# jorge-menjivar/tekken-rs

Measured on AMD Instinct MI355X. Metric: input MB/s tokenized (whole node), higher is better.
Workload: dtype u8

## Files before the change

tekken-rs_amd/csrc/tk_flat_args.h:

```cpp
#ifndef TK_FLAT_ARGS_H
#define TK_FLAT_ARGS_H
#include <stdint.h>

#include "tk_counters.h"
#include "tk_tables.h"

#define TKF_W 32
#define TKF_REGION (64 * TKF_W)
#define TKF_HL 32
#define TKF_HR 64
#define TKF_COMMIT (TKF_REGION - TKF_HL - TKF_HR)
#define TKF_LONGCAP 256u
#define TKF_STRIDE (TKF_COMMIT + 64 + TKF_LONGCAP)
#define TKF_OWN (TKF_COMMIT + TKF_HR)
#define TKF_MISSOFF0 0u
#define TKF_MISSOFF1 (TKF_OWN / 2u)
#define TKF_MISSOFF2 (TKF_MISSOFF1 + (TKF_OWN + 8u) / 9u)
#define TKF_MISSOFF3 (TKF_MISSOFF2 + (TKF_OWN + 16u) / 17u)
#define TKF_MISSCAP ((TKF_MISSOFF3 + (TKF_OWN + 32u) / 33u + 7u) & ~7u)
#define TKF_POSBITS 11
#define TKF_REC(pos, len, slot) ((pos) | ((len) << TKF_POSBITS) | ((slot) << (TKF_POSBITS + 7)))
#define TKF_REC_POS(rec) ((rec) & ((1u << TKF_POSBITS) - 1u))
#define TKF_REC_LEN(rec) (((rec) >> TKF_POSBITS) & 127u)
#define TKF_REC_SLOT(rec) ((rec) >> (TKF_POSBITS + 7))
#define TKF_HOLE 0xFFFFFFFFu

struct TkFlatLongRec {
    uint64_t pos;
    uint32_t chunk;
    uint32_t slot;
    uint32_t len;
    uint32_t reserved;
};

#define TKF_LREC_FRAG 0x80000000u

struct TkFlatArgs {
    const uint8_t* bytes;
    const uint64_t* doc_offs;
    uint64_t n_docs, n_bytes, n_chunks;
    const uint32_t* first_doc;
    uint32_t* tmp;
    uint32_t* kcount;
    uint32_t* lstart;
    uint32_t* miss_list;
    uint32_t* miss_count;
    const uint64_t* miss_prefix;
    uint32_t* wave_first;
    uint32_t* wave_first_wide;
    uint32_t* holes;
    uint32_t* flags;
    TkFlatLongRec* long_recs;
    uint32_t* long_count;
    uint32_t long_cap;
    int long_merge128;
    const uint32_t* long_ctl;
    uint32_t* cut_list;
    const uint32_t* cut_count;
    uint32_t* late_list;
    uint32_t* late_count;
    tk_memo_entry* memo_tab;
    uint32_t memo_mask;
    int memo_probe;
    uint32_t memo_epoch;
    uint32_t* memo_hits;
    tk_memo_entry* memo_log;
    uint32_t* memo_log_counts;
    uint32_t memo_log_per_wave, memo_log_waves;
    uint8_t* dbg_starts;
    int pattern;
    int dbg_ablate;
    TkTablesView t;
};

#endif
```

tekken-rs_amd/csrc/tk_flat_impl.h:

```cpp
#ifndef TK_FLAT_IMPL_H
#define TK_FLAT_IMPL_H
#include <stdint.h>

#include "tk_encode_impl.h"
#include "tk_flat_args.h"

#define TKF_WM 0xFFFFFFFFu
#define TKF_LOGW 5
#define TKF_TOPBIT 0x80000000u
#define TKF_NHL (TKF_HL / TKF_W)
#ifndef TKF_LISTCAP
#define TKF_LISTCAP 1056
#endif
#define TKF_MAXPIECES (TKF_LISTCAP - 2)

#define TKF_L_LIST 0
#define TKF_L_DS (TKF_L_LIST + TKF_LISTCAP / 2)
#define TKF_L_PS (TKF_L_DS + 64)
#define TKF_L_PFX (TKF_L_PS + 64)
#define TKF_L_BAD (TKF_L_PFX + 64)
#define TKF_L_BPFX (TKF_L_BAD + 64)
#define TKF_WALKOFF 192
#define TKF_WALKCAP (2 * (TKF_LISTCAP / 2 - TKF_WALKOFF))
#define TKF_L_CL TKF_L_LIST
#define TKF_L_KM (TKF_L_BPFX + 64)
#define TKF_L_MEMO TKF_L_KM
#define TKF_L_TXT (TKF_L_KM + 17 * 4)
#define TKF_L_CONST (TKF_L_TXT + TKF_REGION / 4 + 4)
#define TKF_LDS_WORDS (TKF_L_CONST + 8)
#define TKF_L_FS TKF_LDS_WORDS
#define TKF_LDS_WORDS_CUT (TKF_LDS_WORDS + 64)


TK_DEV uint32_t tkf_shl(uint32_t x, int k) { return (uint32_t)((((uint64_t)x << 32) | (uint64_t)wv_dn1(x)) >> (32 - k)); }
TK_DEV uint32_t tkf_shr(uint32_t x, int k) { return (uint32_t)((((uint64_t)wv_up1(x) << 32) | (uint64_t)x) >> k); }
TK_DEV uint32_t tkf_shl_any(uint32_t x, int k, int lane) {
    const int q = k >> TKF_LOGW, r = k & (TKF_W - 1);
    const int s1 = lane - q, s2 = lane - q - 1;
    uint32_t v1 = wv_shfl(x, s1 & 63), v2 = wv_shfl(x, s2 & 63);
    if (s1 < 0) v1 = 0;
    if (s2 < 0) v2 = 0;
    return (uint32_t)((((uint64_t)v1 << TKF_W) | (uint64_t)v2) >> (TKF_W - r)) & TKF_WM;
}
TK_DEV uint32_t tkf_shr_any(uint32_t x, int k, int lane) {
    const int q = k >> TKF_LOGW, r = k & (TKF_W - 1);
    const int s1 = lane + q, s2 = lane + q + 1;
    uint32_t v1 = wv_shfl(x, s1 & 63), v2 = wv_shfl(x, s2 & 63);
    if (s1 > 63) v1 = 0;
    if (s2 > 63) v2 = 0;
    return (uint32_t)((((uint64_t)v2 << TKF_W) | (uint64_t)v1) >> r) & TKF_WM;
}
TK_DEV bool tkf_any(uint32_t x) { return wv_ballot(x != 0u) != 0ull; }

TK_DEV uint32_t tkf_add(uint32_t a, uint32_t b) {
    const uint32_t t = a + b;
    const uint64_t G = wv_ballot(t < a);
    const uint64_t P = wv_ballot((t & TKF_WM) == TKF_WM);
    const uint64_t x = G | P;
    const uint64_t cin = (x + G) ^ x ^ G;
    return (t + (wv_inverse_ballot(cin) ? 1u : 0u)) & TKF_WM;
}
TK_DEV uint32_t tkf_ripple(uint32_t run, uint32_t seeds) { return (tkf_add(run, seeds) ^ run) & run; }
TK_DEV uint32_t tkf_land(uint32_t run, uint32_t seeds) { return tkf_add(run, seeds) & ~run & TKF_WM; }

TK_DEV uint32_t tkf_scan_excl(uint32_t v, int lane, uint32_t* total) {
    (void)lane;
    const uint32_t x = wv_scan_incl_u32(v);
    *total = wv_readlane(x, 63);
    return x - v;
}

struct TkfClass {
    uint32_t L, N, S, NL, SP, AP, HI, STMD, RV, E, LL;
    uint32_t U8C, LEAD, C5, BF;
    uint32_t UP, SL, X, M;
    uint32_t F2, F3;
    bool nmb;
};

TK_DEV void tkf_transpose8(uint32_t& lo, uint32_t& hi) {
    uint32_t t;
    t = ((lo >> 7) ^ lo) & 0x00AA00AAu; lo ^= t ^ (t << 7);
    t = ((hi >> 7) ^ hi) & 0x00AA00AAu; hi ^= t ^ (t << 7);
    t = ((lo >> 14) ^ lo) & 0x0000CCCCu; lo ^= t ^ (t << 14);
    t = ((hi >> 14) ^ hi) & 0x0000CCCCu; hi ^= t ^ (t << 14);
    t = (((lo >> 28) | (hi << 4)) ^ lo) & 0xF0F0F0F0u;
    lo ^= t ^ (t << 28);
    hi ^= t >> 4;
}

TK_DEV TkfClass tkf_classify(const uint32_t* x) {
    uint32_t a_lo = x[0], a_hi = x[1], b_lo = x[2], b_hi = x[3];
    tkf_transpose8(a_lo, a_hi);
    tkf_transpose8(b_lo, b_hi);
    uint32_t c_lo = x[4], c_hi = x[5], d_lo = x[6], d_hi = x[7];
    tkf_transpose8(c_lo, c_hi);
    tkf_transpose8(d_lo, d_hi);
    const uint32_t u0 = wv_perm(b_lo, a_lo, 0x05010400u), u1 = wv_perm(b_lo, a_lo, 0x07030602u);
    const uint32_t v0 = wv_perm(d_lo, c_lo, 0x05010400u), v1 = wv_perm(d_lo, c_lo, 0x07030602u);
    const uint32_t p0 = wv_perm(v0, u0, 0x05040100u), p1 = wv_perm(v0, u0, 0x07060302u);
    const uint32_t p2 = wv_perm(v1, u1, 0x05040100u), p3 = wv_perm(v1, u1, 0x07060302u);
    const uint32_t u2 = wv_perm(b_hi, a_hi, 0x05010400u), u3 = wv_perm(b_hi, a_hi, 0x07030602u);
    const uint32_t v2 = wv_perm(d_hi, c_hi, 0x05010400u), v3 = wv_perm(d_hi, c_hi, 0x07030602u);
    const uint32_t p4 = wv_perm(v2, u2, 0x05040100u), p5 = wv_perm(v2, u2, 0x07060302u);
// ... 372 lines not shown
                        } else if (b0b < 0xF0u) {
                            if ((b1 & 0xC0u) == 0x80u && (b2 & 0xC0u) == 0x80u) {
                                cp = ((b0b & 0x0Fu) << 12) | ((b1 & 0x3Fu) << 6) | (b2 & 0x3Fu); clen = 3;
                            }
                        } else if (b0b < 0xF8u) {
                            if ((b1 & 0xC0u) == 0x80u && (b2 & 0xC0u) == 0x80u && (b3 & 0xC0u) == 0x80u) {
                                cp = ((b0b & 0x07u) << 18) | ((b1 & 0x3Fu) << 12) | ((b2 & 0x3Fu) << 6) | (b3 & 0x3Fu); clen = 4;
                            }
                        }
                        const uint32_t q = cp < 0x10000u ? cp : 0u;
                        uint32_t cw = t.uc_bmp[q >> 4];
                        uint32_t cls = (cw >> (2u * (q & 15u))) & 3u;
                        if (cp >= 0x10000u) cls = cp == 0xFFFFFFFFu ? (uint32_t)TK_CLS_O : tk_uc_class(t, cp);
                        if (cls != TK_CLS_O) {
                            const uint32_t wi = p >> TKF_LOGW, sh = p & (TKF_W - 1);
                            const uint64_t bits = (uint64_t)((1u << clen) - 1u) << sh;
                            wv_lds_or(cl + (cls - 1u) * 64u + wi, (uint32_t)(bits & TKF_WM));
                            if ((bits >> TKF_W) && wi < 63u) wv_lds_or(cl + (cls - 1u) * 64u + wi + 1u, (uint32_t)(bits >> TKF_W));
                            if (cls == TK_CLS_N) nmb = true;
                        }
                    }
                }
            }
        }
        while (!dealt && wv_ballot(w != 0u)) {
            if (w) {
                if (PAT) {
                    const int i = __builtin_ctz(w);
                    w &= w - 1u;
                    uint32_t clen;
                    const uint32_t cp = decode(i, &clen);
                    uint32_t cls = TK_CLS_O, extra = 0;
                    if (cp != 0xFFFFFFFFu) {
                        const uint32_t c2 = tk_uc_class2(t, cp);
                        cls = c2 == 1u || c2 == 2u ? TK_CLS_L : c2 == 5u ? TK_CLS_N : c2 == 6u ? TK_CLS_S : TK_CLS_O;
                        extra = c2 == 1u ? 1u : c2 == 3u ? 2u : c2 == 4u ? 3u : 0u;
                    }
                    mark(i, clen, cls, extra);
                } else {
                    const int i0 = __builtin_ctz(w);
                    w &= w - 1u;
                    const bool two = w != 0u;
                    const int i1 = two ? __builtin_ctz(w) : i0;
                    w &= w - 1u;
                    uint32_t l0, l1;
                    const uint32_t cp0 = decode(i0, &l0), cp1 = decode(i1, &l1);
                    const uint32_t q0 = cp0 < 0x10000u ? cp0 : 0u, q1 = cp1 < 0x10000u ? cp1 : 0u;
                    uint32_t w0 = t.uc_bmp[q0 >> 4], w1 = t.uc_bmp[q1 >> 4];
                    WV_PIN(w0); WV_PIN(w1);
                    uint32_t c0 = (w0 >> (2u * (q0 & 15u))) & 3u, c1 = (w1 >> (2u * (q1 & 15u))) & 3u;
                    if (cp0 >= 0x10000u) c0 = cp0 == 0xFFFFFFFFu ? (uint32_t)TK_CLS_O : tk_uc_class(t, cp0);
                    if (cp1 >= 0x10000u) c1 = cp1 == 0xFFFFFFFFu ? (uint32_t)TK_CLS_O : tk_uc_class(t, cp1);
                    mark(i0, l0, c0, 0u);
                    if (two) mark(i1, l1, c1, 0u);
                }
            }
        }
        wv_lds_sync();
        m.L |= cl[lane];
        m.N |= cl[64 + lane];
        m.S |= cl[128 + lane];
        m.nmb = wv_ballot(nmb) != 0ull;
        if (PAT) {
            m.UP |= cl[192 + lane];
            m.X = cl[256 + lane];
            m.M = cl[320 + lane];
        }
    }
    if (TKF_ABL(a, 16)) {
        const uint32_t v = m.L + m.N + m.S + m.NL + m.SP + m.AP + m.HI + m.STMD + m.RV + m.E + m.LL;
        if (lane == 0) {
            a.kcount[c] = v == 0xFFFFFFFFu ? 1u : 0u;
            for (int k = 0; k < 4; ++k) a.miss_count[k * a.n_chunks + c] = 0u;
        }
        return false;
    }

    lds[TKF_L_DS + lane] = 0u;
    lds[TKF_L_BAD + lane] = 0u;
    wv_lds_sync();
    const uint64_t fd = WV_KARGS(TkFlatArgs, a).first_doc[c];
    bool starts_at_r1 = false;
    {
        const auto& ka = WV_KARGS(TkFlatArgs, a);
        for (uint64_t base = fd;; base += 64) {
            const uint64_t d = base + (uint64_t)lane;
            int64_t s = INT64_MAX;
            if (d <= ka.n_docs) s = (int64_t)ka.doc_offs[d];
            const bool in = s < r1;
            if (in) wv_lds_or(lds + TKF_L_DS + ((s - r0) >> TKF_LOGW), 1u << ((s - r0) & (TKF_W - 1)));
            if (s == r1) starts_at_r1 = true;
            if (wv_ballot(in) != ~0ull) break;
        }
        starts_at_r1 = wv_ballot(starts_at_r1) != 0ull;
    }
    wv_lds_sync();
    const uint32_t DS = lds[TKF_L_DS + lane];

    uint32_t SPR, cont;
    uint32_t PS = PAT ? tkf_rules_json(m, DS, lane, &SPR, &cont) : tkf_rules(m, DS, lane, &SPR, &cont);
    if (TKF_ABL(a, 8)) {
        if (lane == 0) {
            a.kcount[c] = (PS + SPR + cont) == 0xFFFFFFFFu ? 1u : 0u;
            for (int k = 0; k < 4; ++k) a.miss_count[k * a.n_chunks + c] = 0u;
        }
        return false;
    }
    if (!CUT && !PAT) {
        const uint64_t Zm = wv_ballot(PS == 0u) & ~(((uint64_t)1 << TKF_NHL) - 1ull);
        if (Zm & (Zm >> 1)) {
            const uint64_t lc = (uint64_t)wv_first(lds[TKF_L_CONST + 6]) | ((uint64_t)wv_first(lds[TKF_L_CONST + 7]) << 32);
            if (lc != 0ull) {
                const uint32_t* ctl = reinterpret_cast<const uint32_t*>(wv_global_ptr(lc));
                const uint64_t lp = (uint64_t)wv_first(ctl[TKC_CTL(TKC_CUT_CTL)]) | ((uint64_t)wv_first(ctl[TKC_CTL(TKC_CUT_CTL_HI)]) << 32);
                if (lp != 0ull) {
                    if (lane == 0) {
                        const uint32_t q = wv_atomic_add(const_cast<uint32_t*>(ctl) + TKC_CTL(TKC_CUT_CHUNKS), 1u);
                        reinterpret_cast<uint32_t*>(const_cast<uint8_t*>(wv_global_ptr(lp)))[q] = (uint32_t)c;
                    }
                    return true;
                }
            }
        }
    }
    uint32_t commit_mask = (uint32_t)(lane - TKF_NHL) < (uint32_t)(TKF_COMMIT / TKF_W) ? TKF_WM : 0u;
    if (cb != TKF_HL + TKF_COMMIT)
        commit_mask = (tkf_lowmask32(cb - TKF_W * lane < 0 ? 0 : cb - TKF_W * lane) & ~tkf_lowmask32(ca - TKF_W * lane < 0 ? 0 : ca - TKF_W * lane)) & TKF_WM;
    if (DBG && a.dbg_starts) {
        for (int k = 0; k < TKF_W; ++k)
            if ((commit_mask >> k) & 1u) a.dbg_starts[r0 + TKF_W * lane + k] = (PS >> k) & 1u;
    }

    uint32_t BAD = 0;
    {
        const uint32_t d0 = wv_readlane(DS, 0);
        const uint32_t n0 = wv_readlane(m.N | (m.U8C & ~(m.U8C + 1u)), 0);
        const uint32_t l0 = wv_readlane((PAT ? (m.NL | m.SL) : m.NL) | (m.U8C & ~(m.U8C + 1u)), 0);
        const bool covered = n0 == TKF_WM || l0 == TKF_WM;
        if (r0 > 0 && d0 == 0u && covered && lane == TKF_NHL) BAD |= 1u;
        if (PAT) {
            const uint32_t lead_cont = m.U8C & ~(m.U8C + 1u);
            const uint32_t wd = m.L | m.X | m.M, om = (TKF_WM & ~(m.L | m.X | m.N | m.S));
            bool cov2 = wv_readlane(wd | lead_cont, 0) == TKF_WM || wv_readlane(om | m.NL | m.SL | lead_cont, 0) == TKF_WM;
            if (r0 > 0 && d0 == 0u && cov2 && lane == TKF_NHL) BAD |= 1u;
        }
        const uint32_t top = wv_readlane(SPR, 63);
        if (r1 < n && (top & TKF_TOPBIT) && !starts_at_r1) {
            const uint32_t nz = ~cont & TKF_WM;
            const uint64_t NZ = wv_ballot(nz != 0u);
            int f = 0;
            if (NZ) {
                const int tl = tk_msb64(NZ);
                const uint32_t w = wv_readlane(nz, tl);
                f = TKF_W * tl + (31 - __builtin_clz(w));
            }
            if (f < cb) {
                const int at = f > ca ? f : ca;
                if (lane == (at >> TKF_LOGW)) BAD |= 1u << (at & (TKF_W - 1));
            }
        }
    }

    uint32_t own_mask = commit_mask;
    uint32_t FS = 0;
    if (CUT) {
        const uint32_t R1 = lane >= TKF_NHL ? (~PS & TKF_WM) : 0u;
        uint32_t F = R1 & tkf_shr(R1, 1);
        F &= tkf_shr(F, 2);
        F &= tkf_shr(F, 4);
        F &= tkf_shr(F, 8);
        F &= tkf_shr(F, 16);
        F &= wv_up1(F);
        const uint32_t S64 = PS & commit_mask & tkf_shr(F, 1);
        uint32_t LM = 0;
        if (tkf_any(S64)) LM = tkf_ripple(R1, tkf_shl(S64, 1) & R1);
        uint32_t f_lo = TKF_REGION;
        {
            const uint64_t Bm = wv_ballot(lane >= TKF_NHL && PS != 0u);
            if (Bm) {
                const int fl = tk_ctz64(Bm);
                f_lo = (uint32_t)TKF_W * (uint32_t)fl + (uint32_t)__builtin_ctz(wv_readlane(PS, fl));
            }
        }
        uint32_t LMc = 0;
        if (f_lo >= (uint32_t)ca + 64u) {
            const int lo = ca - TKF_W * lane, hi = (int)f_lo - TKF_W * lane;
            LMc = tkf_lowmask32(hi < 0 ? 0 : hi) & ~tkf_lowmask32(lo < 0 ? 0 : lo);
            LM |= LMc;
        }
        const uint32_t ge_cb = ~tkf_lowmask32(cb - TKF_W * lane < 0 ? 0 : cb - TKF_W * lane);
        const bool closed = tkf_any(PS & ge_cb);
        const uint32_t need = LM | tkf_shr(LM, 1);
        uint32_t TG = 0, K2 = 0;
        {
            const uint32_t prevb = wv_dn1(x[TKF_W / 4 - 1]) >> 24;
            uint32_t nb = wv_up1(x[0]) & 0xFFu;
            if (lane == 63) nb = nextb;
            if (need) {
                uint32_t b0 = prevb, b1 = x[0] & 0xFFu;
                for (int k = 0; k < TKF_W; ++k) {
                    const uint32_t b2 = k + 1 < TKF_W ? (x[(k + 1) >> 2] >> (8 * ((k + 1) & 3))) & 0xFFu : nb;
                    if ((need >> k) & 1u) {
                        const uint32_t i3 = b0 | (b1 << 8) | (b2 << 16), i2 = b0 | (b1 << 8);
                        TG |= ((a.t.cut_g3[i3 >> 5] >> (i3 & 31u)) & 1u) << k;
                        K2 |= ((a.t.cut_k2[i2 >> 5] >> (i2 & 31u)) & 1u) << k;
                    }
                    b0 = b1; b1 = b2;
                }
            }
        }
        FS = LM & ~PS & ~K2 & ~TG & ~tkf_shl(TG, 1);
        if (tkf_any(LMc)) {
            const uint32_t win = ((uint32_t)lane == (uint32_t)TKF_NHL || (uint32_t)lane == (uint32_t)TKF_NHL + 1u) ? TKF_WM : 0u;
            if (!tkf_any(FS & LMc & win)) { FS &= ~LMc; LM &= ~LMc; }
        }
        PS |= FS;
        if (closed) own_mask |= LM & ge_cb;
        lds[TKF_L_FS + lane] = FS;
    }

    uint32_t PSown = PS & own_mask;
    uint32_t PSlist = lane >= TKF_NHL ? PS : 0u;
    uint32_t np_all, np_own, pfx_all, pfx_own;
    {
        uint32_t tot;
        const uint32_t pf = tkf_scan_excl((uint32_t)__builtin_popcount(PSlist) | ((uint32_t)__builtin_popcount(PSown) << 16), lane, &tot);
        pfx_all = pf & 0xFFFFu; pfx_own = pf >> 16;
        np_all = tot & 0xFFFFu; np_own = tot >> 16;
    }
    const int npass = np_all > TKF_MAXPIECES ? 2 : 1;
    uint32_t* tmp = WV_KARGS(TkFlatArgs, a).tmp + c * TKF_STRIDE;
    uint32_t* mq = WV_KARGS(TkFlatArgs, a).miss_list + c * TKF_MISSCAP;
    uint32_t E = 0;
    uint32_t base_own = 0;
    uint32_t nm0 = 0, nm1 = 0, nm2 = 0, nm3 = 0;
    uint32_t lane_lo = TKF_NHL, lane_hi = 64;
    auto doc_outputs = [&](bool want_flags, bool anybad) {
        const uint64_t dfirst = fd > 0 ? fd - 1 : 0;
        const auto& ka = WV_KARGS(TkFlatArgs, a);
        for (uint64_t base = dfirst;; base += 64) {
            const uint64_t d = base + (uint64_t)lane;
            int64_t s = INT64_MAX, e = INT64_MAX;
            if (d < ka.n_docs) {
                s = (int64_t)ka.doc_offs[d];
                e = (int64_t)ka.doc_offs[d + 1];
            }
            const bool in = s < c1;
            if (in && s >= c0) {
                const uint32_t p = (uint32_t)(s - r0);
                const uint32_t pl = p >> TKF_LOGW;
                if (npass == 1 || (pl >= lane_lo && pl < lane_hi)) {
                    const uint32_t pi = lds[TKF_L_PFX + pl] + (uint32_t)__builtin_popcount(lds[TKF_L_PS + pl] & ((1u << (p & (TKF_W - 1))) - 1u));
                    ka.lstart[d] = pi < np_own ? list[pi] : base_own + np_own + E;
                }
            }
            if (want_flags && anybad && in && e > c0) {
                const int64_t lo = s > r0 ? s - r0 : 0, hi = e < r1 ? e - r0 : TKF_REGION;
                if (hi > lo) {
                    const uint32_t pl = (uint32_t)lo, ph = (uint32_t)hi;
                    const uint32_t cl = lds[TKF_L_BPFX + (pl >> TKF_LOGW)] + (uint32_t)__builtin_popcount(lds[TKF_L_BAD + (pl >> TKF_LOGW)] & ((1u << (pl & (TKF_W - 1))) - 1u));
                    uint32_t ch;
                    if (ph >= TKF_REGION) ch = lds[TKF_L_BPFX + 63] + (uint32_t)__builtin_popcount(lds[TKF_L_BAD + 63]);
                    else ch = lds[TKF_L_BPFX + (ph >> TKF_LOGW)] + (uint32_t)__builtin_popcount(lds[TKF_L_BAD + (ph >> TKF_LOGW)] & ((1u << (ph & (TKF_W - 1))) - 1u));
                    if (ch > cl) ka.flags[d] = 1u;
                }
            }
            if (wv_ballot(in) != ~0ull) break;
        }
    };
  for (int pass = 0; pass < npass; ++pass) {
    uint32_t sentinel = TKF_REGION;
    if (npass == 2) {
        lane_lo = pass ? 32 : TKF_NHL;
        lane_hi = pass ? 64 : 32;
        const bool mine = (uint32_t)lane >= lane_lo && (uint32_t)lane < lane_hi;
        PSlist = mine ? PS : 0u;
        PSown = PSlist & own_mask;
        uint32_t tot;
        const uint32_t pf = tkf_scan_excl((uint32_t)__builtin_popcount(PSlist) | ((uint32_t)__builtin_popcount(PSown) << 16), lane, &tot);
        pfx_all = pf & 0xFFFFu; pfx_own = pf >> 16;
        np_all = tot & 0xFFFFu; np_own = tot >> 16;
        if (pass == 0) {
            const uint64_t Bm = wv_ballot(lane >= 32 && PS != 0u);
            if (Bm) {
                const int fl = (int)__builtin_ctzll(Bm);
                sentinel = (uint32_t)TKF_W * (uint32_t)fl + (uint32_t)__builtin_ctz(wv_readlane(PS, fl));
            }
        }
    }
    {
        uint32_t w = PSlist, idx = pfx_all;
        while (wv_ballot(w != 0u)) {
            if (w) {
                list[idx++] = (uint16_t)(TKF_W * lane + __builtin_ctz(w));
                w &= w - 1u;
            }
        }
        if (lane == 0) list[np_all] = (uint16_t)sentinel;
    }
    lds[TKF_L_PS + lane] = PSown;
    lds[TKF_L_PFX + lane] = pfx_own;
    wv_lds_sync();

    const uint32_t nbatch = (np_own + 63u) / 64u;
    for (uint32_t j = 0; j < nbatch; ++j) {
        const uint32_t idx = j * 64u + (uint32_t)lane;
        const bool act = idx < np_own;
        uint32_t pos, len;
        if (j + 1u < nbatch) {
            const uint32_t p0 = list[idx], p1 = list[idx + 1u];
            pos = p0;
            len = p1 - p0;
        } else {
// ... 5 lines not shown
        {
            const uint32_t* tw = lds + TKF_L_TXT + (pos >> 2);
            const uint32_t t0 = tw[0], t1 = tw[1], t2 = tw[2], t3 = tw[3], t4 = tw[4];
            const uint32_t sh = pos & 3u;
            const uint32_t* km = lds + TKF_L_KM + 4u * (len < 16u ? len : 16u);
            kk[0] = wv_alignbyte(t1, t0, sh) & km[0]; kk[1] = wv_alignbyte(t2, t1, sh) & km[1];
            kk[2] = wv_alignbyte(t3, t2, sh) & km[2]; kk[3] = wv_alignbyte(t4, t3, sh) & km[3];
        }
        uint32_t r = kk[0];
        uint32_t h = 0;
        if (TKF_ABL(a, 1)) {
            r = 7u;
        } else if (TKF_ABL(a, 64)) {
            r = (kk[0] ^ kk[1] ^ kk[2] ^ kk[3]) & 0xFFFFu;
        } else {
            h = tk_key_hash((uint32_t)MODE, kk[0], kk[1], kk[2], kk[3], len);
            if (TKF_ABL(a, 128)) {
                r = h & 0xFFFFu;
            } else if (len - 2u <= 14u) {
                const uint32_t* kc = lds + TKF_L_CONST;
                const uint64_t b8 = (uint64_t)kc[2] | ((uint64_t)kc[3] << 32), b16 = (uint64_t)kc[4] | ((uint64_t)kc[5] << 32);
                r = tk_probe_key_h(wv_global_ptr(b8), TKF_ABL(a, 512) ? kc[0] >> 4 : kc[0], wv_global_ptr(b16), TKF_ABL(a, 512) ? kc[1] >> 4 : kc[1],
                                   h, kk[0], kk[1], kk[2], kk[3], len);
            }
        }
        bool frag = false;
        if (CUT) {
            const uint32_t pe = pos + len;
            frag = act && ((((lds[TKF_L_FS + (pos >> TKF_LOGW)] >> (pos & (TKF_W - 1))) & 1u) != 0u) ||
                           (pe < (uint32_t)TKF_REGION && ((lds[TKF_L_FS + (pe >> TKF_LOGW)] >> (pe & (TKF_W - 1))) & 1u) != 0u));
            if (frag && len >= 2u) r = TK_RANK_MAX;
        }
        bool toolong = false;
        if (wv_ballot(len > 16u)) {
            uint32_t lres = 0;
            bool lopen = false;
            if (len > 64u) {
                lopen = idx + 1u == np_all && sentinel == TKF_REGION && r0 + (int64_t)TKF_REGION < (int64_t)a.n_bytes;
                const bool have_ctl = (lds[TKF_L_CONST + 6] | lds[TKF_L_CONST + 7]) != 0u;
                if (!PAT && have_ctl && (lopen || len <= TKF_LONGCAP) && !(CUT && frag && lopen)) lres = lopen ? TKF_LONGCAP : len;
                else toolong = true;
            } else if (len > 16u && !TKF_ABL(a, 1) && !(CUT && frag)) {
                r = TK_RANK_MAX;
                const uint32_t pb = tk_k64_prebit(h);
                const uint32_t* pre = reinterpret_cast<const uint32_t*>(t.key64_tab + t.key64_mask + 1u);
                const bool maybe = TKF_ABL(a, 64) || TKF_ABL(a, 128) || ((pre[pb >> 5] >> (pb & 31u)) & 1u) != 0u;
                if (maybe) r = tk_probe_key64(t, lds + TKF_L_TXT + (pos >> 2), pos & 3u, len, kk[0], kk[1], kk[2], kk[3]);
            }
            if (toolong) wv_lds_or(lds + TKF_L_BAD + (pos >> TKF_LOGW), 1u << (pos & (TKF_W - 1)));
            if (wv_ballot(lres != 0u)) {
                const bool longp = lres != 0u;
                const bool lmiss = r == TK_RANK_MAX && !toolong && !longp && !TKF_ABL(a, 2);
                uint32_t lslot = base_own + idx + E;
                {
                    uint32_t tot;
                    lslot += tkf_scan_excl(lmiss ? len - 1u : longp ? lres - 1u : 0u, lane, &tot);
                    E += tot;
                }
                {
                    const uint64_t LB = wv_ballot(longp);
                    const int lfirst = tk_ctz64(LB);
                    const uint32_t* ctl = reinterpret_cast<const uint32_t*>(wv_global_ptr((uint64_t)lds[TKF_L_CONST + 6] | ((uint64_t)lds[TKF_L_CONST + 7] << 32)));
                    uint32_t qbase = 0;
                    if (lane == lfirst) qbase = wv_atomic_add(const_cast<uint32_t*>(ctl) + TKC_CTL(TKC_LONG_RECS), (uint32_t)tk_popc64(LB));
                    qbase = wv_shfl(qbase, lfirst);
                    const uint32_t q = qbase + (uint32_t)tk_popc64(LB & tk_lowmask(lane));
                    TkFlatLongRec* recs = reinterpret_cast<TkFlatLongRec*>(const_cast<uint8_t*>(wv_global_ptr((uint64_t)ctl[TKC_CTL(TKC_LONG_CTL)] | ((uint64_t)ctl[TKC_CTL(TKC_LONG_CTL_HI)] << 32))));
                    if (!longp) {
                    } else if (q < ctl[TKC_CTL(TKC_LONG_CTL_CAP)]) {
                        TkFlatLongRec lr;
                        lr.pos = (uint64_t)(r0 + (int64_t)pos); lr.chunk = (uint32_t)c; lr.slot = lslot; lr.len = lopen ? 0u : (CUT && frag ? len | TKF_LREC_FRAG : len); lr.reserved = lres;
                        recs[q] = lr;
                    } else {
                        wv_lds_or(lds + TKF_L_BAD + (pos >> TKF_LOGW), 1u << (pos & (TKF_W - 1)));
                    }
                }
                if (wv_ballot(lmiss)) {
                    const uint32_t cls = (len > 8u ? 1u : 0u) + (len > 16u ? 1u : 0u) + (len > 32u ? 1u : 0u);
                    const uint32_t sh = cls * 8u;
                    uint32_t ctot;
                    const uint32_t before = (tkf_scan_excl(lmiss ? 1u << sh : 0u, lane, &ctot) >> sh) & 0xFFu;
                    if (lmiss) {
                        const uint32_t qb = cls == 0u ? TKF_MISSOFF0 + nm0 : cls == 1u ? TKF_MISSOFF1 + nm1 : cls == 2u ? TKF_MISSOFF2 + nm2 : TKF_MISSOFF3 + nm3;
                        mq[qb + before] = TKF_REC(pos, len, lslot);
                    }
                    nm0 += ctot & 0xFFu;
                    nm1 += (ctot >> 8) & 0xFFu;
                    nm2 += (ctot >> 16) & 0xFFu;
                    nm3 += ctot >> 24;
                }
                wv_lds_sync();
                if (act) {
                    list[idx] = (uint16_t)lslot;
                    if (!lmiss && !longp && !TKF_ABL(a, 4)) tmp[lslot] = r + t.num_special;
                }
                continue;
            }
        }
        const bool miss = r == TK_RANK_MAX && !toolong && !TKF_ABL(a, 2);
        uint32_t slot = base_own + idx + E;
        const uint64_t MB = wv_ballot(miss);
        uint32_t res = len;
        bool mhit = false;
        uint32_t mv0 = 0, mv1 = 0, mv2 = 0, mv4 = 0;
        if (MB) {
            const uint64_t mbase = MEMO ? (uint64_t)wv_first(lds[TKF_L_MEMO + 0]) | ((uint64_t)wv_first(lds[TKF_L_MEMO + 1]) << 32) : 0ull;
            if (MEMO && mbase != 0ull) {
                if (miss && len <= 16u) {
                    const uint32_t ms = tk_memo_slot(h) & lds[TKF_L_MEMO + 2];
                    const tk_u32x4* me = reinterpret_cast<const tk_u32x4*>(wv_global_ptr(mbase) + ((uint64_t)ms << 5));
                    tk_u32x4 ek = me[0], ev = me[1];
                    WV_PIN(ek.x); WV_PIN(ev.x);
                    if ((((ek.x ^ kk[0]) | (ek.y ^ kk[1]) | (ek.z ^ kk[2]) | (ek.w ^ kk[3])) == 0u) && tk_memo_len(ev.w) == len) {
                        mhit = true;
                        res = tk_memo_n(ev.w);
                        mv0 = ev.y; mv1 = ev.z; mv2 = ev.w; mv4 = ev.x;
                    }
                }
                const uint64_t HB = wv_ballot(mhit);
                if (HB && lane == 0) lds[TKF_L_MEMO + 3] += (uint32_t)tk_popc64(HB);
            }
            if ((MB & (MB - 1ull)) == 0ull) {
                const int src = tk_ctz64(MB);
                const uint32_t extra = wv_readlane(res, src) - 1u;
                if (lane > src) slot += extra;
                E += extra;
            } else {
                uint32_t tot;
                slot += tkf_scan_excl(miss ? res - 1u : 0u, lane, &tot);
                E += tot;
            }
            const bool qmiss = MEMO ? miss && !mhit : miss;
            const uint64_t QB = wv_ballot(qmiss);
            if (QB == 0ull) {
            } else if (wv_ballot(qmiss && len > 8u) == 0ull) {
                if (qmiss) mq[TKF_MISSOFF0 + nm0 + (uint32_t)tk_popc64(QB & tk_lowmask(lane))] = TKF_REC(pos, len, slot);
                nm0 += (uint32_t)tk_popc64(QB);
            } else {
                const uint32_t cls = (len > 8u ? 1u : 0u) + (len > 16u ? 1u : 0u) + (len > 32u ? 1u : 0u);
                const uint32_t sh = cls * 8u;
                uint32_t ctot;
                const uint32_t before = (tkf_scan_excl(qmiss ? 1u << sh : 0u, lane, &ctot) >> sh) & 0xFFu;
                if (qmiss) {
                    const uint32_t qb = cls == 0u ? TKF_MISSOFF0 + nm0 : cls == 1u ? TKF_MISSOFF1 + nm1 : cls == 2u ? TKF_MISSOFF2 + nm2 : TKF_MISSOFF3 + nm3;
                    mq[qb + before] = TKF_REC(pos, len, slot);
                }
                nm0 += ctot & 0xFFu;
                nm1 += (ctot >> 8) & 0xFFu;
                nm2 += (ctot >> 16) & 0xFFu;
                nm3 += ctot >> 24;
            }
        }
        wv_lds_sync();
        if (act) {
            list[idx] = (uint16_t)slot;
            if (!miss && !TKF_ABL(a, 4)) tmp[slot] = r + t.num_special;
        }
        if (MEMO && mhit) {
            tmp[slot] = tk_memo_id(mv4, mv0, mv1, mv2, 0u) + t.num_special;
            if (res > 1u) tmp[slot + 1u] = tk_memo_id(mv4, mv0, mv1, mv2, 1u) + t.num_special;
            if (res > 2u) tmp[slot + 2u] = tk_memo_id(mv4, mv0, mv1, mv2, 2u) + t.num_special;
            if (res > 3u) tmp[slot + 3u] = tk_memo_id(mv4, mv0, mv1, mv2, 3u) + t.num_special;
            if (res > 4u) tmp[slot + 4u] = tk_memo_id(mv4, mv0, mv1, mv2, 4u) + t.num_special;
        }
    }
    if (pass + 1 < npass) {
        wv_lds_sync();
        doc_outputs(false, false);
        base_own += np_own;
        wv_lds_sync();
    }
  }
    if (lane == 0) {
        const auto& ka = WV_KARGS(TkFlatArgs, a);
        ka.kcount[c] = base_own + np_own + E;
        ka.miss_count[c] = nm0;
        ka.miss_count[ka.n_chunks + c] = nm1;
        ka.miss_count[2 * ka.n_chunks + c] = nm2;
        ka.miss_count[3 * ka.n_chunks + c] = nm3;
    }

    BAD |= lds[TKF_L_BAD + lane];
    const bool anybad = tkf_any(BAD);
    if (anybad) {
        uint32_t nb;
        const uint32_t bp = tkf_scan_excl((uint32_t)__builtin_popcount(BAD), lane, &nb);
        lds[TKF_L_BAD + lane] = BAD;
        lds[TKF_L_BPFX + lane] = bp;
    }
    wv_lds_sync();
    doc_outputs(true, anybad);
    wv_lds_sync();
    return false;
}

TK_DEV void tk_flat_long_wave(const TkFlatArgs& a, const TkPolyPow& pw, uint32_t q, int lane, uint32_t* scratch) {
    const TkFlatLongRec lr = a.long_recs[q];
    const uint64_t g = lr.pos;
    uint64_t d = a.first_doc[lr.chunk];
    d = d > 0 ? d - 1 : 0;
    while (d + 1 < a.n_docs && a.doc_offs[d + 1] <= g) ++d;
    d = wv_first64(d);
    if (wv_first(a.flags[d]) != 0u) return;
    TkEncodeArgs ea;
    ea.bytes = a.bytes; ea.doc_offs = a.doc_offs; ea.n_docs = a.n_docs; ea.staging = nullptr; ea.counts = nullptr;
    ea.work_counter = nullptr; ea.defer_count = nullptr; ea.defer_list = nullptr; ea.todo_list = nullptr; ea.n_todo = 0; ea.n_todo_dev = nullptr;
    ea.scratch = scratch; ea.scratch_words_per_wave = 0; ea.add_bos = 0; ea.add_eos = 0; ea.split_only = 0; ea.pattern = 0; ea.dbg_ablate = 0;
    ea.dbg_starts = nullptr; ea.dbg_mark = nullptr; ea.long_list = nullptr; ea.long_count = nullptr; ea.long_min = 0; ea.long_lazy_mul = 0; ea.long_force = 0;
    ea.long_jobs = nullptr; ea.long_job_count = nullptr; ea.long_job_cap = 0; ea.t = a.t;
    const uint64_t s1 = wv_first64(a.doc_offs[d + 1]);
    const bool frag = (lr.len & TKF_LREC_FRAG) != 0u;
    const uint32_t rlen = lr.len & ~TKF_LREC_FRAG;
    const uint64_t e = rlen ? g + rlen : wv_first64(tk_match_end(a.t, a.bytes, g, s1));
    const uint32_t len = (uint32_t)(e - g);
    uint32_t* out = a.tmp + (uint64_t)lr.chunk * TKF_STRIDE + lr.slot;
    if (e - g > (uint64_t)lr.reserved) {
        if (lane == 0) {
            if (a.late_list) {
                if (wv_atomic_exch(a.flags + d, 1u) == 0u) a.late_list[wv_atomic_add(a.late_count, 1u)] = (uint32_t)d;
            } else {
                a.flags[d] = 1u;
            }
        }
        return;
    }
    uint32_t cur = 0;
    const uint32_t r = frag ? TK_RANK_MAX : tk_piece_lookup(ea, pw, lane, g, e);
    if (r != TK_RANK_MAX) {
// ... 208 lines not shown
                const uint32_t j = tkm_ctz(above);
                const alive_t above2 = tkm_clear_lowest(above);
                const alive_t below = alive & tkm_low(bi, (const alive_t*)nullptr);
                const bool has_next = tkm_any(above2), has_prev = tkm_any(below);
                const uint32_t k = has_next ? tkm_ctz(above2) : 0u;
                const uint32_t p = has_prev ? tkm_msb(below) : 0u;
                const uint32_t tn = tok_at(k, alive), tp = tok_at(p, alive);
                alive = alive & ~tkm_bit(j, (const alive_t*)nullptr);
                keyc[j * 64] = 0xFFFFFFFFu;
                if (C) keyc[(bi + 1u) * 64] = DEAD | rank;
                else tokc[bi * 64] = rank;
                uint32_t r_next = TK_RANK_MAX, r_prev = TK_RANK_MAX;
                tk_probe_pair_x2f(t, filt, has_next, rank, tn, has_prev, tp, rank, r_next, r_prev);
                keyc[bi * 64] = r_next == TK_RANK_MAX ? 0xFFFFFFFFu : ((r_next << PB) | bi);
                if (has_prev) keyc[p * 64] = r_prev == TK_RANK_MAX ? 0xFFFFFFFFu : ((r_prev << PB) | p);
            }
        }
    }
    const uint32_t np = tkm_popc(alive);
    if (!C && ml != nullptr) {
        bool ins = mine && np <= TK_MEMO_MAXIDS;
        uint32_t k[4] = {0u, 0u, 0u, 0u};
        tk_memo_entry* slot = nullptr;
        if (wv_ballot(ins) && ml->n < ml->cap) {
            if (ins) {
#pragma unroll
                for (int q = 0; q < 4; ++q) {
                    const int keep = (int)len - 4 * q;
                    k[q] = (q < N / 4 && keep > 0) ? (kk[q < N / 4 ? q : 0] & (keep >= 4 ? 0xFFFFFFFFu : ((1u << (8 * keep)) - 1u))) : 0u;
                }
                slot = a.memo_tab + (tk_memo_slot(tk_key_hash(t.key_hash_mode, k[0], k[1], k[2], k[3], len)) & a.memo_mask);
                if (a.memo_probe == 0u) {
                    const uint32_t cw = slot->w4;
                    if (cw != 0u && (cw & TK_MEMO_TAG) == 0u) ins = false;
                }
            }
        }
        const uint64_t IB = wv_ballot(ins);
        if (IB && ml->n < ml->cap) {
            const uint32_t at = ml->n + (uint32_t)tk_popc64(IB & tk_lowmask(lane));
            if (ins && at < ml->cap) {
                uint32_t r5[5] = {0u, 0u, 0u, 0u, 0u};
                alive_t rem = alive;
#pragma unroll
                for (int q = 0; q < 5; ++q) {
                    if ((uint32_t)q < np) r5[q] = tokc[tkm_ctz(rem) * 64u];
                    rem = tkm_clear_lowest(rem);
                }
                uint32_t v[3], w4;
                tk_memo_pack(r5, np, len, &w4, v);
                tk_memo_entry* w = ml->base + at;
                wv_store16(w->k, k[0], k[1], k[2], k[3]);
                wv_store16(&w->w4, w4, v[0], v[1], v[2]);
                slot->w4 = (uint32_t)(w - a.memo_log);
            }
            const uint32_t nn = ml->n + (uint32_t)tk_popc64(IB);
            ml->n = nn < ml->cap ? nn : ml->cap;
        }
    }
    if (mine && !TKM_AB(a, 256)) {
        alive_t rem = alive;
#pragma unroll
        for (int q0 = 0; q0 < N; q0 += 4) {
            uint32_t v[4];
#pragma unroll
            for (int q = 0; q < 4; ++q) {
                const uint32_t pos = tkm_any(rem) ? tkm_ctz(rem) : 0u;
                const uint32_t id = tok_at(pos, alive) + t.num_special;
                v[q] = (uint32_t)(q0 + q) < np ? id : TKF_HOLE;
                rem = tkm_clear_lowest(rem);
            }
            if ((uint32_t)q0 + 4u <= len) {
                wv_store16(out + q0, v[0], v[1], v[2], v[3]);
            } else {
                if ((uint32_t)q0 < len) out[q0] = v[0];
                if ((uint32_t)q0 + 1u < len) out[q0 + 1] = v[1];
                if ((uint32_t)q0 + 2u < len) out[q0 + 2] = v[2];
            }
        }
    }
    return mine ? len - np : 0u;
}

TK_DEV void tk_merge_holes(const TkFlatArgs& a, bool have, uint32_t holes, uint32_t chunk, int64_t g, int lane) {
    if (wv_ballot(have && holes != 0u) && !TKM_AB(a, 512)) {
        uint64_t d = 0;
        if (have) {
            d = a.first_doc[chunk];
            d = d > 0 ? d - 1 : 0;
            for (;;) {
                const uint64_t i1 = d + 1 < a.n_docs ? d + 1 : a.n_docs, i2 = d + 2 < a.n_docs ? d + 2 : a.n_docs;
                const uint64_t i3 = d + 3 < a.n_docs ? d + 3 : a.n_docs, i4 = d + 4 < a.n_docs ? d + 4 : a.n_docs;
                uint64_t o1 = a.doc_offs[i1], o2 = a.doc_offs[i2], o3 = a.doc_offs[i3], o4 = a.doc_offs[i4];
                const uint32_t cnt = ((int64_t)o1 <= g ? 1u : 0u) + ((int64_t)o2 <= g ? 1u : 0u) + ((int64_t)o3 <= g ? 1u : 0u) + ((int64_t)o4 <= g ? 1u : 0u);
                d += cnt;
                if (cnt < 4u) break;
            }
        }
        const uint32_t key = have ? (uint32_t)d : 0xFFFFFFFFu;
        const uint32_t kprev = wv_shfl(key, lane > 0 ? lane - 1 : 0), knext = wv_shfl(key, lane < 63 ? lane + 1 : 63);
        const bool head = lane == 0 || kprev != key, tail = lane == 63 || knext != key;
        const uint64_t HEADS = wv_ballot(head);
        const uint32_t P = wv_scan_incl_u32(have ? holes : 0u);
        const int start = tk_msb64(HEADS & (tk_lowmask(lane) | (1ull << lane)));
        const uint32_t before = wv_shfl(P, start > 0 ? start - 1 : 0);
        const uint32_t sum = P - (start > 0 ? before : 0u);
        if (have && tail && sum) wv_atomic_add(a.holes + d, sum);
    }
}

TK_DEV void tk_merge_items64(const TkFlatArgs& a, bool have, uint32_t rec, uint32_t chunk, int lane, uint32_t* mlds, const uint32_t* filt) {
    const uint32_t pos = TKF_REC_POS(rec), len = TKF_REC_LEN(rec), slot = TKF_REC_SLOT(rec);
    const int64_t g = (int64_t)chunk * TKF_COMMIT - TKF_HL + (int64_t)pos;
    uint32_t* out = a.tmp + (uint64_t)chunk * TKF_STRIDE + slot;
    uint32_t kk[16];
    for (int q = 0; q < 16; ++q) kk[q] = 0u;
    if (have) {
        if (g + 64 <= (int64_t)a.n_bytes) {
            wv_load16(a.bytes + g, kk);
            wv_load16(a.bytes + g + 16, kk + 4);
            wv_load16(a.bytes + g + 32, kk + 8);
            wv_load16(a.bytes + g + 48, kk + 12);
        } else {
            for (uint32_t q = 0; q < len; ++q) kk[q >> 2] |= (uint32_t)a.bytes[g + q] << (8 * (q & 3));
        }
    }
    uint32_t holes = 0;
    if (wv_ballot(have)) holes = tk_merge_lds<64>(a, filt, have, kk, len, out, mlds, lane);
    tk_merge_holes(a, have, holes, chunk, g, lane);
}

template <int N>
TK_DEV void tk_merge_long_wave(const TkFlatArgs& a, uint64_t wave_id, int lane, uint32_t* mlds, const uint32_t* filt) {
    const uint64_t n = *a.long_count < a.long_cap ? *a.long_count : a.long_cap;
    const uint64_t item = wave_id * 64 + (uint64_t)lane;
    if (wave_id * 64 >= n) return;
    TkFlatLongRec lr;
    lr.pos = 0; lr.chunk = 0; lr.slot = 0; lr.len = 0; lr.reserved = 0;
    if (item < n) lr = a.long_recs[item];
    const bool have = (lr.reserved & 0x80000000u) != 0u && lr.len <= (uint32_t)N && lr.len > (uint32_t)N / 2u;
    lr.reserved &= 0x3FFFFFFFu;
    if (wv_ballot(have) == 0ull) return;
    const int64_t g = (int64_t)lr.pos;
    uint32_t* out = a.tmp + (uint64_t)lr.chunk * TKF_STRIDE + lr.slot;
    uint32_t kk[N / 4];
    for (int q = 0; q < N / 4; ++q) kk[q] = 0u;
    if (have) {
        if (g + N <= (int64_t)a.n_bytes) {
#pragma unroll
            for (int q = 0; q < N / 16; ++q) wv_load16(a.bytes + g + 16 * q, kk + 4 * q);
        } else {
            for (uint32_t q = 0; q < lr.len; ++q) kk[q >> 2] |= (uint32_t)a.bytes[g + q] << (8 * (q & 3));
        }
    }
    uint32_t holes = tk_merge_lds<N>(a, filt, have, kk, lr.len, out, mlds, lane);
    if (have) {
        for (uint32_t k = lr.len; k < lr.reserved; ++k) out[k] = TKF_HOLE;
        holes += lr.reserved - lr.len;
    }
    tk_merge_holes(a, have, holes, lr.chunk, g, lane);
}

template <bool WIDE>
TK_DEV void tk_merge_items(const TkFlatArgs& a, bool have, uint32_t rec, uint32_t chunk, int lane, uint32_t* mlds, const uint32_t* filt, TkMemoLog* ml) {
    const TkTablesView& t = a.t;
    const uint32_t pos = TKF_REC_POS(rec), len = TKF_REC_LEN(rec), slot = TKF_REC_SLOT(rec);
    const int64_t g = (int64_t)chunk * TKF_COMMIT - TKF_HL + (int64_t)pos;
    uint32_t* out = a.tmp + (uint64_t)chunk * TKF_STRIDE + slot;
    uint32_t holes = 0;

    {
        const uint32_t cap = WIDE ? 32u : TKM_SHORT;
        const bool inregs = have && len <= cap;
        uint32_t kk[WIDE ? 8 : 4];
        for (int q = 0; q < (WIDE ? 8 : 4); ++q) kk[q] = 0u;
        if (inregs) {
            if (g + (int64_t)cap <= (int64_t)a.n_bytes) {
                wv_load16(a.bytes + g, kk);
                if (WIDE) wv_load16(a.bytes + g + 16, kk + 4);
            } else {
                for (uint32_t q = 0; q < len; ++q) kk[q >> 2] |= (uint32_t)a.bytes[g + q] << (8 * (q & 3));
            }
        }
        if (!WIDE) {
            const bool s8 = inregs && len <= 8u, s16 = inregs && len > 8u;
            if (wv_ballot(s8)) holes += tk_merge_lds<8>(a, filt, s8, kk, len, out, mlds, lane, ml);
            if (wv_ballot(s16)) holes += tk_merge_lds<16>(a, filt, s16, kk, len, out, mlds, lane, ml);
        } else {
            if (wv_ballot(inregs)) holes += tk_merge_lds<32>(a, filt, inregs, kk, len, out, mlds, lane);
        }
    }

    uint64_t LONGM = wv_ballot(have && len > (WIDE ? 32u : TKM_SHORT));
    while (LONGM) {
        const int src = tk_ctz64(LONGM);
        LONGM &= LONGM - 1ull;
        const uint32_t plen = wv_shfl(len, src);
        const uint32_t glo = wv_shfl((uint32_t)g, src), ghi = wv_shfl((uint32_t)((uint64_t)g >> 32), src);
        const int64_t pg = (int64_t)(((uint64_t)ghi << 32) | glo);
        const uint32_t pchunk = wv_shfl(chunk, src), pslot = wv_shfl(slot, src);
        uint32_t* pout = a.tmp + (uint64_t)pchunk * TKF_STRIDE + pslot;
        const int pe = (int)plen;
        const bool inmiss = lane < pe;
        const uint32_t b0 = inmiss ? (uint32_t)a.bytes[pg + lane] : 0u;
        const uint32_t b1 = wv_up1(b0);
        uint64_t A = wv_ballot(inmiss);
        uint32_t tok = b0;
        uint32_t prank = TK_RANK_MAX;
        if (inmiss && lane + 1 < pe) prank = t.pair2[b0 | (b1 << 8)];
        for (int round = 0; round < 64; ++round) {
            const uint32_t key = prank == TK_RANK_MAX ? 0xFFFFFFFFu : ((prank << 6) | (uint32_t)lane);
            const uint32_t segmin = wv_min_u32(key);
            if (segmin == 0xFFFFFFFFu) break;
            const bool winner = key == segmin;
            const uint64_t Wm = wv_ballot(winner);
            const bool alive = tk_bit(A, lane);
            const uint64_t below = A & tk_lowmask(lane);
            const bool dead = alive && below && tk_bit(Wm, tk_msb64(below));
            const uint64_t Dm = wv_ballot(dead);
            A &= ~Dm;
            if (winner) tok = prank;
            if (dead) prank = TK_RANK_MAX;
            const uint64_t z = lane < 63 ? (A >> (lane + 1)) : 0ull;
            const int na = z ? lane + 1 + tk_ctz64(z) : 64;
            const bool has_next = na < pe;
            const uint32_t tn = wv_shfl(tok, na < 64 ? na : lane);
            const bool need = tk_bit(A, lane) && (winner || (has_next && tk_bit(Wm, na)));
            if (need) prank = has_next ? tk_probe_pair_f(t, filt, tok, tn) : TK_RANK_MAX;
        }
        const uint32_t k = (uint32_t)tk_popc64(A);
        if (inmiss && tk_bit(A, lane)) pout[tk_popc64(A & tk_lowmask(lane))] = tok + t.num_special;
        if (inmiss && (uint32_t)lane >= k) pout[lane] = TKF_HOLE;
        if (lane == src) holes = plen - k;
    }

    tk_merge_holes(a, have, holes, chunk, g, lane);
}

TK_DEV bool tk_memo_log_live(const uint32_t* counts, uint32_t per_wave, uint32_t i) { return i % per_wave < counts[i / per_wave]; }
TK_DEV uint32_t tk_memo_slot_of(const tk_memo_entry& r, uint32_t key_hash_mode, uint32_t mask) {
    return tk_memo_slot(tk_key_hash(key_hash_mode, r.k[0], r.k[1], r.k[2], r.k[3], tk_memo_len(r.v[2]))) & mask;
}
TK_DEV void tk_memo_commit_one(tk_memo_entry* tab, const tk_memo_entry* log, uint32_t i, uint32_t key_hash_mode, uint32_t mask) {
    const tk_memo_entry r = log[i];
    tk_memo_entry* w = tab + tk_memo_slot_of(r, key_hash_mode, mask);
    if (w->w4 == i) {
        wv_store16(w->k, r.k[0], r.k[1], r.k[2], r.k[3]);
        wv_store16(&w->w4, r.w4, r.v[0], r.v[1], r.v[2]);
    }
}

#endif
```

Before: 395,000.

## Encode document rank in miss-queue records to skip doc search in merge

```diff
diff --git a/tekken-rs_amd/csrc/tk_flat_args.h b/tekken-rs_amd/csrc/tk_flat_args.h
--- a/tekken-rs_amd/csrc/tk_flat_args.h
+++ b/tekken-rs_amd/csrc/tk_flat_args.h
@@ -19,10 +19,15 @@
 #define TKF_MISSOFF3 (TKF_MISSOFF2 + (TKF_OWN + 16u) / 17u)
 #define TKF_MISSCAP ((TKF_MISSOFF3 + (TKF_OWN + 32u) / 33u + 7u) & ~7u)
 #define TKF_POSBITS 11
-#define TKF_REC(pos, len, slot) ((pos) | ((len) << TKF_POSBITS) | ((slot) << (TKF_POSBITS + 7)))
+#define TKF_LENBITS 6
+#define TKF_SLOTBITS 12
+#define TKF_RANK_SEARCH 7u
+#define TKF_REC(pos, len, slot, rank) \
+    ((pos) + ((len) << TKF_POSBITS) + ((slot) << (TKF_POSBITS + TKF_LENBITS)) + ((rank) << (TKF_POSBITS + TKF_LENBITS + TKF_SLOTBITS)))
 #define TKF_REC_POS(rec) ((rec) & ((1u << TKF_POSBITS) - 1u))
-#define TKF_REC_LEN(rec) (((rec) >> TKF_POSBITS) & 127u)
-#define TKF_REC_SLOT(rec) ((rec) >> (TKF_POSBITS + 7))
+#define TKF_REC_LEN(rec) (((((rec) >> TKF_POSBITS) - 1u) & ((1u << TKF_LENBITS) - 1u)) + 1u)
+#define TKF_REC_SLOT(rec) (((((rec) >> TKF_POSBITS) - 1u) >> TKF_LENBITS) & ((1u << TKF_SLOTBITS) - 1u))
+#define TKF_REC_RANK(rec) ((rec) >> (TKF_POSBITS + TKF_LENBITS + TKF_SLOTBITS))
 #define TKF_HOLE 0xFFFFFFFFu
 
 struct TkFlatLongRec {
diff --git a/tekken-rs_amd/csrc/tk_flat_impl.h b/tekken-rs_amd/csrc/tk_flat_impl.h
--- a/tekken-rs_amd/csrc/tk_flat_impl.h
+++ b/tekken-rs_amd/csrc/tk_flat_impl.h
@@ -13,6 +13,8 @@
 #define TKF_LISTCAP 1056
 #endif
 #define TKF_MAXPIECES (TKF_LISTCAP - 2)
+static_assert(TKF_REGION <= (1u << TKF_POSBITS) && TKF_STRIDE + 1u < (1u << TKF_SLOTBITS) && TKF_POSBITS + TKF_LENBITS + TKF_SLOTBITS == 29,
+              "queue record (tk_flat_args.h): position, length - 1 (a length of 64 carries into the slot), slot, three rank bits");
 
 #define TKF_L_LIST 0
 #define TKF_L_DS (TKF_L_LIST + TKF_LISTCAP / 2)
@@ -20,6 +22,7 @@
 #define TKF_L_PFX (TKF_L_PS + 64)
 #define TKF_L_BAD (TKF_L_PFX + 64)
 #define TKF_L_BPFX (TKF_L_BAD + 64)
+#define TKF_L_RKPFX TKF_L_BPFX
 #define TKF_WALKOFF 192
 #define TKF_WALKCAP (2 * (TKF_LISTCAP / 2 - TKF_WALKOFF))
 #define TKF_L_CL TKF_L_LIST
@@ -558,6 +561,7 @@
     const uint64_t fd = WV_KARGS(TkFlatArgs, a).first_doc[c];
     bool starts_at_r1 = false;
     {
+        uint32_t rk_starts = 0;
         const auto& ka = WV_KARGS(TkFlatArgs, a);
         for (uint64_t base = fd;; base += 64) {
             const uint64_t d = base + (uint64_t)lane;
@@ -566,9 +570,13 @@
             const bool in = s < r1;
             if (in) wv_lds_or(lds + TKF_L_DS + ((s - r0) >> TKF_LOGW), 1u << ((s - r0) & (TKF_W - 1)));
             if (s == r1) starts_at_r1 = true;
-            if (wv_ballot(in) != ~0ull) break;
+            const uint64_t IN = wv_ballot(in);
+            rk_starts += (uint32_t)tk_popc64(IN);
+            if (IN != ~0ull) break;
         }
         starts_at_r1 = wv_ballot(starts_at_r1) != 0ull;
+        if (CUT || fd == 0 || rk_starts >= TKF_RANK_SEARCH) rk_starts = 0xFFFFFFFFu;
+        if (lane == 0) lds[TKF_L_RKPFX] = rk_starts;
     }
     wv_lds_sync();
     const uint32_t DS = lds[TKF_L_DS + lane];
@@ -697,14 +705,24 @@
 
     uint32_t PSown = PS & own_mask;
     uint32_t PSlist = lane >= TKF_NHL ? PS : 0u;
-    uint32_t np_all, np_own, pfx_all, pfx_own;
+    uint32_t np_all, np_own, pfx_all, pfx_own, rk_pfx;
+    bool rk_ok;
     {
+        const uint32_t rk_starts = lds[TKF_L_RKPFX];
         uint32_t tot;
-        const uint32_t pf = tkf_scan_excl((uint32_t)__builtin_popcount(PSlist) | ((uint32_t)__builtin_popcount(PSown) << 16), lane, &tot);
-        pfx_all = pf & 0xFFFFu; pfx_own = pf >> 16;
-        np_all = tot & 0xFFFFu; np_own = tot >> 16;
+        const uint32_t pf = tkf_scan_excl((uint32_t)__builtin_popcount(PSlist) | ((uint32_t)__builtin_popcount(PSown) << 16) |
+                                          ((uint32_t)__builtin_popcount(DS) << 28), lane, &tot);
+        pfx_all = pf & 0xFFFFu; pfx_own = (pf >> 16) & 0xFFFu;
+        np_all = tot & 0xFFFFu; np_own = (tot >> 16) & 0xFFFu;
+        rk_pfx = pf >> 28;
+        rk_ok = (tot >> 28) == rk_starts;
     }
     const int npass = np_all > TKF_MAXPIECES ? 2 : 1;
+    if (!rk_ok || npass == 2) {
+        lds[TKF_L_DS + lane] = 0u;
+        rk_pfx = TKF_RANK_SEARCH;
+    }
+    lds[TKF_L_RKPFX + lane] = rk_pfx;
     uint32_t* tmp = WV_KARGS(TkFlatArgs, a).tmp + c * TKF_STRIDE;
     uint32_t* mq = WV_KARGS(TkFlatArgs, a).miss_list + c * TKF_MISSCAP;
     uint32_t E = 0;
@@ -876,7 +894,7 @@
                     const uint32_t before = (tkf_scan_excl(lmiss ? 1u << sh : 0u, lane, &ctot) >> sh) & 0xFFu;
                     if (lmiss) {
                         const uint32_t qb = cls == 0u ? TKF_MISSOFF0 + nm0 : cls == 1u ? TKF_MISSOFF1 + nm1 : cls == 2u ? TKF_MISSOFF2 + nm2 : TKF_MISSOFF3 + nm3;
-                        mq[qb + before] = TKF_REC(pos, len, lslot);
+                        mq[qb + before] = TKF_REC(pos, len, lslot, TKF_RANK_SEARCH);
                     }
                     nm0 += ctot & 0xFFu;
                     nm1 += (ctot >> 8) & 0xFFu;
@@ -926,9 +944,14 @@
             }
             const bool qmiss = MEMO ? miss && !mhit : miss;
             const uint64_t QB = wv_ballot(qmiss);
+            uint32_t rank = 0;
+            if (QB != 0ull) {
+                const uint32_t pl = pos >> TKF_LOGW;
+                rank = lds[TKF_L_RKPFX + pl] + (uint32_t)__builtin_popcount(lds[TKF_L_DS + pl] << (31u - (pos & (TKF_W - 1))));
+            }
             if (QB == 0ull) {
             } else if (wv_ballot(qmiss && len > 8u) == 0ull) {
-                if (qmiss) mq[TKF_MISSOFF0 + nm0 + (uint32_t)tk_popc64(QB & tk_lowmask(lane))] = TKF_REC(pos, len, slot);
+                if (qmiss) mq[TKF_MISSOFF0 + nm0 + (uint32_t)tk_popc64(QB & tk_lowmask(lane))] = TKF_REC(pos, len, slot, rank);
                 nm0 += (uint32_t)tk_popc64(QB);
             } else {
                 const uint32_t cls = (len > 8u ? 1u : 0u) + (len > 16u ? 1u : 0u) + (len > 32u ? 1u : 0u);
@@ -937,7 +960,7 @@
                 const uint32_t before = (tkf_scan_excl(qmiss ? 1u << sh : 0u, lane, &ctot) >> sh) & 0xFFu;
                 if (qmiss) {
                     const uint32_t qb = cls == 0u ? TKF_MISSOFF0 + nm0 : cls == 1u ? TKF_MISSOFF1 + nm1 : cls == 2u ? TKF_MISSOFF2 + nm2 : TKF_MISSOFF3 + nm3;
-                    mq[qb + before] = TKF_REC(pos, len, slot);
+                    mq[qb + before] = TKF_REC(pos, len, slot, rank);
                 }
                 nm0 += ctot & 0xFFu;
                 nm1 += (ctot >> 8) & 0xFFu;
@@ -1312,12 +1335,16 @@
     return mine ? len - np : 0u;
 }
 
-TK_DEV void tk_merge_holes(const TkFlatArgs& a, bool have, uint32_t holes, uint32_t chunk, int64_t g, int lane) {
+TK_DEV void tk_merge_holes(const TkFlatArgs& a, bool have, uint32_t holes, uint32_t chunk, int64_t g, int lane, uint32_t rank) {
     if (wv_ballot(have && holes != 0u) && !TKM_AB(a, 512)) {
         uint64_t d = 0;
         if (have) {
             d = a.first_doc[chunk];
             d = d > 0 ? d - 1 : 0;
+        }
+        if (have && rank != TKF_RANK_SEARCH) {
+            d += rank;
+        } else if (have) {
             for (;;) {
                 const uint64_t i1 = d + 1 < a.n_docs ? d + 1 : a.n_docs, i2 = d + 2 < a.n_docs ? d + 2 : a.n_docs;
                 const uint64_t i3 = d + 3 < a.n_docs ? d + 3 : a.n_docs, i4 = d + 4 < a.n_docs ? d + 4 : a.n_docs;
@@ -1357,7 +1384,7 @@
     }
     uint32_t holes = 0;
     if (wv_ballot(have)) holes = tk_merge_lds<64>(a, filt, have, kk, len, out, mlds, lane);
-    tk_merge_holes(a, have, holes, chunk, g, lane);
+    tk_merge_holes(a, have, holes, chunk, g, lane, TKF_REC_RANK(rec));
 }
 
 template <int N>
@@ -1388,7 +1415,7 @@
         for (uint32_t k = lr.len; k < lr.reserved; ++k) out[k] = TKF_HOLE;
         holes += lr.reserved - lr.len;
     }
-    tk_merge_holes(a, have, holes, lr.chunk, g, lane);
+    tk_merge_holes(a, have, holes, lr.chunk, g, lane, TKF_RANK_SEARCH);
 }
 
 template <bool WIDE>
@@ -1464,7 +1491,7 @@
         if (lane == src) holes = plen - k;
     }
 
-    tk_merge_holes(a, have, holes, chunk, g, lane);
+    tk_merge_holes(a, have, holes, chunk, g, lane, TKF_REC_RANK(rec));
 }
 
 TK_DEV bool tk_memo_log_live(const uint32_t* counts, uint32_t per_wave, uint32_t i) { return i % per_wave < counts[i / per_wave]; }
```

New measurement: 389,200. -1.5%, worse.
